# imperatormk/candle-birefnet

Measured on AMD Instinct MI355X. Metric: images/sec @1024x1024 Swin-L, higher is better.
Workload: dtype f32 storage+accumulate; GEMM operands as two fp16 planes of the power-of-two-scaled operand (22-bit mantissa), 3 fp16 MFMAs/product (fp32-equivalent inside the fp16 range: |GEMM input| < 8190); 1 GPU; BASELINE configs[1]: Swin-L 1024x1024 batch=1 fp32 on 1xMI355X (single-image latency); batch_per_gpu=1, global_batch=1, size=1024, deform_mode=reference_cpu, compute=f32_half2, streams_per_gpu=1, branch_streams_per_gpu=5, inputs=resident in HBM (torch cuda tensors), weights: synthetic seed 42

## Files before the change

candle_birefnet_amd/csrc/brn_graph_swin.cpp:

```cpp
#include "brn_graph.h"

namespace brn {

void swin_stage_dims(int H, int W, int patch, int hs[4], int ws[4]) {
    int h = (H + patch - 1) / patch, w = (W + patch - 1) / patch;
    for (int i = 0; i < 4; ++i) {
        hs[i] = h; ws[i] = w;
        h = (h + 1) / 2; w = (w + 1) / 2;
    }
}

static bool swin_attention_multi(Ctx& c, const SwinBlockW& blk, const float* xn, int B, int nin, const int* hs, const int* wsz, int C, int shift, float* y,
                                 const float* residual, int p2 = 0, int window = 12, const LNW* ln2 = nullptr, float* xn2 = nullptr, int ld_xn2 = 0) {
    const size_t mk = c.arena->mark();
    int M = 0;
    for (int k = 0; k < nin; ++k) M += B * hs[k] * wsz[k];
    float* qkv = c.act_alloc((size_t)M * 3 * C);
    const int ldp = p2 ? C * p2 / 2 : C;
    float* att = c.act_alloc((size_t)M * ldp);
    run_gemm(c, blk.qkv, GemmIO(xn, M, ldp).to(qkv, 3 * C).planes(p2, 0));
    if (!c.dry) {
        WindowAttnParams ps[2]{};
        size_t off = 0;
        double nwin = 0.0;
        for (int k = 0; k < nin; ++k) {
            WindowAttnParams& p = ps[k];
            p.qkv = c.at(qkv, off * 3 * C); p.qkv_bias = blk.qkv.bias; p.rel_table = blk.rel_table; p.out = c.at(att, off * ldp);
            p.io_bf16 = c.bf16;
            p.B = B; p.H = hs[k]; p.W = wsz[k]; p.C = C; p.heads = blk.heads;
            p.Hp = roundup(hs[k], window); p.Wp = roundup(wsz[k], window);
            p.ws = window;
            p.shift = shift; p.scale = 1.0f / sqrtf(32.0f);
            p.planes = (!c.bf16 && window == 12 && (blk.qkv.planes == 2 || blk.qkv.planes == 1)) ? blk.qkv.planes : 0;
            p.h2 = (p.planes == 2 && blk.qkv.half && switches().h2_att) ? 1 : 0;
            if (blk.qkv.half && !p.h2) p.planes = 0;
            p.out_planes = p2;
            p.out_h2 = (p2 == 2 && blk.qkv.half) ? c.h2_scale : 0.f;
            nwin += (double)B * (p.Hp / window) * (p.Wp / window) * blk.heads;
            off += (size_t)B * hs[k] * wsz[k];
        }
        const double ntok = (double)window * window;
        Bracket b(c, FAM_ATTENTION, nwin * 2.0 * 2.0 * ntok * ntok * 32, (double)c.esz() * ((double)M * 4 * C), M, C, shift);
        BRN_LAUNCH(launch_window_attention2(ps[0], nin > 1 ? &ps[1] : nullptr, c.stream));
    }
    bool ln_done = false;
    if (ln2 && xn2 && !p2 && y == residual) ln_done = linear_residual_ln(c, blk.proj, att, M, ldp, y, *ln2, xn2, ld_xn2);
    if (!ln_done) run_gemm(c, blk.proj, GemmIO(att, M, ldp).to(y, C).add(residual, C).planes(p2, 0).f32(c.bf16, c.bf16));
    c.arena->release(mk);
    return ln_done;
}

void swin_attention(Ctx& c, const SwinBlockW& blk, const float* xn, int B, int H, int W, int C, int shift, float* y, const float* residual, int window) {
    swin_attention_multi(c, blk, xn, B, 1, &H, &W, C, shift, y, residual, 0, window);
}

void swin_forward_multi(Ctx& c, const SwinW& w, const SwinIn* ins, int nin, int B, bool outs_f32) {
    if (nin < 1 || nin > 2) fail(BRN_ERR_INVALID_ARG, "swin_forward_multi: 1 or 2 inputs");
    int hs[2][4], wsz[2][4];
    for (int k = 0; k < nin; ++k) swin_stage_dims(ins[k].H, ins[k].W, w.patch, hs[k], wsz[k]);
    auto rows = [&](int k, int i) { return B * hs[k][i] * wsz[k][i]; };
    auto total = [&](int i) { int m = 0; for (int k = 0; k < nin; ++k) m += rows(k, i); return m; };
    const size_t mk0 = c.arena->mark();
    const int E = w.embed_dim;
    float* x = c.arena->alloc((size_t)total(0) * E);
    const int pe_env = switches().patch_ln;
    bool pe_fused = c.bf16 && pe_env != 0 && w.patch_proj.w && w.patch_proj.mode == GEMM_GATHER_NCHW && w.patch_proj.pad == 0 && w.patch_proj.dil == 1 &&
                    w.patch_proj.kh == w.patch_proj.kw && w.patch_norm.C == E && w.patch_norm.g && w.patch_norm.b;
    for (int k = 0; k < nin && pe_fused; ++k)
// ... 100 lines not shown
```

candle_birefnet_amd/csrc/brn_host.h:

```cpp
#pragma once
#include <hip/hip_runtime.h>
#include <stdint.h>
#include <stdarg.h>
#include <string>
#include <deque>
#include <vector>
#include <unordered_map>
#include <stdexcept>
#include <mutex>
#include <type_traits>
#include "../../include/birefnet_hip.h"
#include "brn_kernels.h"

namespace brn {

struct Error : std::runtime_error {
    int code;
    Error(int c, const std::string& m) : std::runtime_error(m), code(c) {}
};
[[noreturn]] void fail(int code, const char* fmt, ...);
void set_last_error(const std::string& s);
#define BRN_HIP(call)                                                                                   \
    do {                                                                                                \
        hipError_t e_ = (call);                                                                         \
// ... 34 lines not shown
    std::vector<hipEvent_t>* event_pool; size_t* event_next;
    int bf16 = 0;
    float h2_scale = 0.f;
    int region = REGION_NONE;
    BranchSet* br = nullptr;
    unsigned pending = 0;
    unsigned br_mask = ~0u;
    int esz() const { return bf16 ? 2 : 4; }
    float* act_alloc(size_t elems) { return arena->alloc_bytes(elems * (size_t)esz()); }
    template <class T> T* at(T* p, size_t elems) const { return reinterpret_cast<T*>(reinterpret_cast<char*>(const_cast<typename std::remove_const<T>::type*>(p)) + elems * (size_t)esz()); }
};

struct Map {
    float* p = nullptr;
    int B = 0, H = 0, W = 0, C = 0, ld = 0, coff = 0;
    Map() = default;
    Map(float* p_, int B_, int H_, int W_, int C_) : p(p_), B(B_), H(H_), W(W_), C(C_), ld(C_) {}
    size_t pixels() const { return (size_t)B * H * W; }
    Map window(int c0, int c) const { Map m = *this; m.coff = coff + c0; m.C = c; return m; }
};
Map new_map(Ctx& c, int B, int H, int W, int C);
static inline int roundup(int x, int m) { return (x + m - 1) / m * m; }

#define BRN_SWITCHES(X)                                                                                                                        \
    X(split_streams,    "BRN_SPLIT_STREAMS",     2,  "sub-batch streams of a device-resident batch (at least two images per part; 1 = one stream)") \
    X(branch_streams,   "BRN_BRANCH_STREAMS",    -1, "-1 = auxiliary branch streams when the batch is one part; 0 = none; else the mask forced (7 ASPP, 8 image-patch, 16 lateral)") \
    X(cu_partition,     "BRN_CU_PARTITION",      0,  "1 / 2 = two sub-batch streams confined to half the CUs of every XCD / to four XCDs each") \
    X(wstat,            "BRN_WSTAT",             3,  "mask of the K served by gemm_wstat_bf16_kernel (1 = 192, 2 = 384)")                     \
    X(wstat_ln,         "BRN_WSTAT_LN",          1,  "0 = stage-0 projection and norm2 as two launches instead of gemm_wstat_ln_bf16_kernel")   \
    X(rowln,            "BRN_ROWLN",             0,  "mask of the widths whose projection + LayerNorm run on gemm_rowln_bf16_kernel (1 = 768, 2 = 384)") \
    X(patch_ln,         "BRN_PATCH_LN",          1,  "0 = PatchEmbed as gather GEMM + LayerNorm in the 16-bit modes too; 2 = fused without the first block's norm1") \
    X(p1_f32,           "BRN_P1_F32",            1,  "0 = the decoder's last map p1 is a 16-bit map like every other in the 16-bit modes")     \
    X(h2_att,           "BRN_H2_ATT",            1,  "0 = mode f32_half2 runs the fp32-MFMA attention kernel instead of the fp16-pair one")     \
    X(h2_ascale,        "BRN_H2_ASCALE",         3,  "log2 of the scale of GEMM input activations before the fp16 split of mode f32_half2 (0 .. 8)") \
    X(deform_f32,       "BRN_DEFORM_F32_KERNEL", 0,  "1 = the 16-bit modes run deformable convolutions on the fp32-MFMA gather kernel")        \
    X(planes_kernel,    "BRN_PLANES_KERNEL",     0,  "1 = split modes with P-layout A on the LDS-DMA plane kernel (diag build only)")           \
    X(conv_chunk_major, "BRN_CONV_CHUNK_MAJOR",  1,  "0 = tap-major K order of the 16-bit implicit-GEMM conv weights (read when weights are packed)") \
    X(offmod_pad8,      "BRN_OFFMOD_PAD8",       1,  "0 = the offset / modulator conv's N padded to 4 instead of 8")
struct Switches {
#define BRN_X(field, name, dflt, doc) int field = dflt;
    BRN_SWITCHES(BRN_X)
#undef BRN_X
};
const Switches& switches();

constexpr int BUILD_BF16 = 16;
constexpr int BUILD_HALF2 = 18;
struct WeightBuild {
    int planes = 0;
    bool f16 = false;
};


struct GemmW {
    float* w = nullptr;
    void* wp = nullptr;
    int planes = 0, wp_rows = 0;
    int half = 0;
    float w_scale = 1.f;
    void* wb = nullptr;
    int wb_rows = 0, wb_ld = 0;
    int wb_chunk_major = 0;
    void* wf = nullptr;
    int N = 0, K = 0, Kreal = 0;
    int Cin = 0, Cinp = 0, kh = 1, kw = 1, stride = 1, pad = 0, dil = 1;
    int mode = GEMM_DENSE;
// ... 187 lines not shown
```

candle_birefnet_amd/csrc/brn_kernels.h:

```cpp
#pragma once
#include <hip/hip_runtime.h>
#include <stdint.h>

namespace brn {

enum GemmMode {
    GEMM_DENSE = 0,
    GEMM_CONV_NHWC = 1,
    GEMM_GATHER_NCHW = 2,
    GEMM_DEFORM_NHWC = 3
};
enum Act { ACT_NONE = 0, ACT_RELU = 1, ACT_GELU_ERF = 2 };

struct GemmParams {
    const float* A;
    const float* W;
    float* C;
    int M, N, K;
    int mode;
    int lda;
    int a_coff;
    int Hin, Win, Cin, kh, kw, stride, pad, dil, Hout, Wout;
    int Kreal;
    const float* om; int om_ld; int om_mask_off;
// ... 63 lines not shown
hipError_t launch_lds_mfma_probe(int blocks, int iters, int np, int variant, float* sink, hipStream_t s);
hipError_t launch_mfma_peak_bf16(int blocks, int iters, float* sink, unsigned long long* clk, int nacc, hipStream_t s);
hipError_t launch_mfma_peak(int blocks, int iters, float* sink, unsigned long long* clk, hipStream_t s);
#endif

struct LayerNormParams {
    const float* x; float* y;
    int rows, C;
    const float* gamma; const float* beta; float eps;
    int ldx;
    int ldy, y_coff;
    int mode; int H, W, Cin;
    int y_planes;
    float y_h2;
    int y_bf16;
};
hipError_t launch_layernorm(const LayerNormParams& p, hipStream_t s);

struct WindowAttnParams {
    const float* qkv;
    const float* qkv_bias;
    const float* rel_table;
    float* out;
    int B, H, W, C, heads;
    int Hp, Wp;
    int shift;
    float scale;
    int planes;
    int out_planes;
    int h2;
    float out_h2;
    int ws;
    int io_bf16;
};
hipError_t launch_window_attention(const WindowAttnParams& p, hipStream_t s);
hipError_t launch_window_attention2(const WindowAttnParams& p, const WindowAttnParams* p2, hipStream_t s);

hipError_t launch_resize_nhwc(const float* x, int B, int Hin, int Win, int C, int ldx, int x_coff,
                              float* y, int Hout, int Wout, int ldy, int y_coff, hipStream_t s, int bf16 = 0, int accumulate = 0);
hipError_t launch_resize_nchw(const float* x, int BC, int Hin, int Win, float* y, int Hout, int Wout, hipStream_t s);
hipError_t launch_nchw_to_nhwc(const float* x, int B, int C, int H, int W, float* y, int ldy, int y_coff, hipStream_t s, int bf16 = 0);
hipError_t launch_nhwc_to_nchw(const float* x, int B, int C, int H, int W, int ldx, int x_coff, float* y, hipStream_t s, int bf16 = 0);
hipError_t launch_image2patches(const float* x, int B, int Cimg, int H, int W, int th, int tw,
                                float* y, int ldy, int cpad, hipStream_t s, int bf16 = 0);
size_t gap_scratch_floats(int B, int HW, int C);
hipError_t launch_gap_nhwc(const float* x, int B, int HW, int C, int ldx, int x_coff, float* scratch, float* out, hipStream_t s, int bf16 = 0);
hipError_t launch_small_fc(const float* x, int B, int Cin, const float* w, int ldw, int w_off, int N,
                           const float* scale, const float* shift, int act, float* y, hipStream_t s);
hipError_t launch_gdt_gate(float* p, int npix, int C, int ldp, int p_coff, const float* g, int ldg,
                           const float* w, float bias, hipStream_t s, int bf16 = 0);
hipError_t launch_pixel_dot(const float* x, int npix, int C, int ldx, int x_coff, const float* w, float bias,
                            float* y, hipStream_t s, int bf16 = 0);
hipError_t launch_f32_to_bf16(const float* x, size_t n, float* y_bf16, hipStream_t s, int f16 = 0);
hipError_t launch_bf16_to_f32(const float* x_bf16, size_t n, float* y, hipStream_t s, int f16 = 0);
hipError_t launch_final_head(const float* q, int B, int h, int w, const float* t, float bias, int H, int W,
                             int apply_sigmoid, float* out, hipStream_t s);
hipError_t launch_head_stencil5x5(const float* img, int B, int H, int W, const float* k, const float* bias, float* y, hipStream_t s);
hipError_t launch_resample_v_u8(const unsigned char* in, int h, int w, int C, int nh, const int* left, const int* count,
                                const float* wts, int max_taps, float* out, hipStream_t s);
hipError_t launch_resample_h(const float* in, int nh, int w, int C, int nw, const int* left, const int* count, const float* wts,
                             int max_taps, unsigned char* out_u8, float* out_f32, const float* mean, const float* stdv, hipStream_t s);
hipError_t launch_mask_u8(const float* logits, long n, int apply_sigmoid, unsigned char* out, hipStream_t s);
hipError_t launch_sigmoid(const float* x, size_t n, float* y, hipStream_t s);
hipError_t launch_mod_sigmoid2(float* x, size_t rows, int ld, int c0, int c1, hipStream_t s);

}
// ... 1 lines not shown
```

candle_birefnet_amd/csrc/kernels/window_attention.hip:

```cpp
#include "../brn_kernels.h"
#include "split_planes.h"
#include <cstdlib>
#include <type_traits>

namespace brn {

typedef float f32x4 __attribute__((ext_vector_type(4)));

constexpr int WS = 12;
constexpr int NTOK = 144;
constexpr int HD = 32;
constexpr int KV_LD = 36;
constexpr int ATT_THREADS = 192;

template <int IOB>
__device__ __forceinline__ f32x4 att_load4(const float* base, long off) {
    if constexpr (IOB != 0) {
        using E = std::conditional_t<IOB == 2, _Float16, __bf16>;
        typedef E ex4_ld __attribute__((ext_vector_type(4)));
        const ex4_ld h = *reinterpret_cast<const ex4_ld*>(reinterpret_cast<const E*>(base) + off);
        return f32x4{(float)h[0], (float)h[1], (float)h[2], (float)h[3]};
    } else return *reinterpret_cast<const f32x4*>(base + off);
}
template <int IOB>
__device__ __forceinline__ f32x4 att_bias4(const float* bias) {
    f32x4 v = *reinterpret_cast<const f32x4*>(bias);
    if constexpr (IOB != 0) {
        using E = std::conditional_t<IOB == 2, _Float16, __bf16>;
#pragma unroll
        for (int e = 0; e < 4; ++e) v[e] = (float)(E)v[e];
    }
    return v;
}
template <int WSZ, int NWV = 3, int IOB = 0>
// ... 136 lines not shown
                o0 = __builtin_amdgcn_mfma_f32_16x16x4f32(vp[0], st[kt][r], o0, 0, 0, 0);
                o1 = __builtin_amdgcn_mfma_f32_16x16x4f32(vp[16], st[kt][r], o1, 0, 0, 0);
            }
            if (kt % 2 == 1) __builtin_amdgcn_sched_barrier(0);
        }
        if (qsrc >= 0 && qtok < NTOK) {
            const float inv = 1.0f / sum;
            if (p.out_planes == 3) {
                float* orow = p.out + (long)qsrc * (C + C / 2);
                store_planes<3>(orow, head * HD + g * 4, o0 * inv);
                store_planes<3>(orow, head * HD + 16 + g * 4, o1 * inv);
            } else if (p.out_planes == 2) {
                float* orow = p.out + (long)qsrc * C;
                store_planes_h(orow, head * HD + g * 4, o0 * inv, p.out_h2);
                store_planes_h(orow, head * HD + 16 + g * 4, o1 * inv, p.out_h2);
            } else if constexpr (IOB != 0) {
                using E = std::conditional_t<IOB == 2, _Float16, __bf16>;
                typedef E ex4_st __attribute__((ext_vector_type(4)));
                E* op = reinterpret_cast<E*>(p.out) + (long)qsrc * C + head * HD + g * 4;
                ex4_st h0, h1;
#pragma unroll
                for (int e = 0; e < 4; ++e) { h0[e] = (E)(o0[e] * inv); h1[e] = (E)(o1[e] * inv); }
                *reinterpret_cast<ex4_st*>(op) = h0;
                *reinterpret_cast<ex4_st*>(op + 16) = h1;
            } else {
                float* op = p.out + (long)qsrc * C + head * HD + g * 4;
                *reinterpret_cast<f32x4*>(op) = o0 * inv;
                *reinterpret_cast<f32x4*>(op + 16) = o1 * inv;
            }
        }
    }
}

typedef __bf16 bf16x8 __attribute__((ext_vector_type(8)));
typedef __bf16 bf16x4 __attribute__((ext_vector_type(4)));
typedef __bf16 bf16x2 __attribute__((ext_vector_type(2)));
constexpr int VT_LD = 148;

__device__ __forceinline__ int kswz(int key) { return (0x78 >> (2 * ((key >> 2) & 3))) & 3; }

constexpr float ATT_H_QKV = 8.0f, ATT_H_P = 2048.0f;
template <int NP, bool H = false>
__global__ void __launch_bounds__(ATT_THREADS) __attribute__((amdgpu_waves_per_eu(3, 3))) window_attention_split_kernel(const WindowAttnParams pa, const WindowAttnParams pb, const int nblk0) {
    static_assert(!H || NP == 2, "fp16 planes come in pairs");
    const bool second = (int)blockIdx.x >= nblk0;
    const WindowAttnParams& p = second ? pb : pa;
    __shared__ __attribute__((aligned(16))) __bf16 Kp[NP * NTOK * HD];
    __shared__ __attribute__((aligned(16))) __bf16 Vt[NP * HD * VT_LD];
    constexpr int TABN = (2 * WS - 1) * (2 * WS - 1);
    __shared__ float tab_s[TABN];
    __shared__ unsigned char rid_s[NTOK];
    __shared__ __attribute__((aligned(16))) float qb_s[HD];

    const int tid = threadIdx.x, lane = tid & 63, wave = tid >> 6;
    const int li = lane & 15, g = lane >> 4;
    const int head = blockIdx.y;
    const int nWw = p.Wp / WS, nW = (p.Hp / WS) * nWw;
    const int bw = second ? (int)blockIdx.x - nblk0 : (int)blockIdx.x;
    const int b = bw / nW, w = bw - b * nW;
    const int wr = w / nWw, wc = w - wr * nWw;
    const int C = p.C, C3 = 3 * C;
    const bool has_mask = p.shift > 0 && (wr == p.Hp / WS - 1 || wc == nWw - 1);

    auto tok_src = [&](int t) {
        const int ti = t / WS, tj = t - ti * WS;
        int sh = wr * WS + ti + p.shift, sw = wc * WS + tj + p.shift;
        if (sh >= p.Hp) sh -= p.Hp;
        if (sw >= p.Wp) sw -= p.Wp;
        return (sh < p.H && sw < p.W) ? (b * p.H + sh) * p.W + sw : -1;
    };
    static_assert((NTOK / 2) * 8 == 3 * ATT_THREADS && ATT_THREADS % 8 == 0 && 3 * ATT_THREADS >= TABN, "three staging items and three table words per thread");
    const int c4 = (tid & 7) * 4;
    const float* kbp = p.qkv_bias + C + head * HD + c4;
    const f32x4 kbias = *reinterpret_cast<const f32x4*>(kbp);
    const f32x4 vbias = *reinterpret_cast<const f32x4*>(kbp + C);
    f32x4 kvr[3][2], vvr[3][2];
    int ssrc[3][2];
#pragma unroll
    for (int it = 0; it < 3; ++it) {
#pragma unroll
        for (int u = 0; u < 2; ++u) {
            const int src = tok_src(((tid >> 3) + it * (ATT_THREADS / 8)) * 2 + u);
            ssrc[it][u] = src;
            const float* kp = p.qkv + (long)max(src, 0) * C3 + C + head * HD + c4;
            kvr[it][u] = *reinterpret_cast<const f32x4*>(kp);
            vvr[it][u] = *reinterpret_cast<const f32x4*>(kp + C);
        }
    }
    float tbw[3];
#pragma unroll
    for (int j = 0; j < 3; ++j) tbw[j] = p.rel_table[head * TABN + min(tid + j * ATT_THREADS, TABN - 1)];
    const float* qbp = p.qkv_bias + head * HD + g * 8;
    const f32x4 qbias0 = *reinterpret_cast<const f32x4*>(qbp);
    const f32x4 qbias1 = *reinterpret_cast<const f32x4*>(qbp + 4);
    int qsrc_n;
    f32x4 qn0, qn1;
    auto load_q = [&](int qtok) {
        qsrc_n = tok_src(qtok);
        const float* qp = p.qkv + (long)max(qsrc_n, 0) * C3 + head * HD + g * 8;
        qn0 = *reinterpret_cast<const f32x4*>(qp);
        qn1 = *reinterpret_cast<const f32x4*>(qp + 4);
    };
    load_q(wave * 16 + li);

    if (tid < NTOK) {
        const int ti = tid / WS, tj = tid - ti * WS;
        const int ph = wr * WS + ti, pw = wc * WS + tj;
        const int fh = ph < p.Hp - WS ? 0 : (ph < p.Hp - p.shift ? 1 : 2);
        const int fw = pw < p.Wp - WS ? 0 : (pw < p.Wp - p.shift ? 1 : 2);
        rid_s[tid] = (unsigned char)(fh * 3 + fw);
    }

#pragma unroll
    for (int it = 0; it < 3; ++it) {
        const int tp = (tid >> 3) + it * (ATT_THREADS / 8);
        f32x4 kv[2], vv[2];
#pragma unroll
        for (int u = 0; u < 2; ++u) {
            kv[u] = ssrc[it][u] < 0 ? kbias : kvr[it][u];
            vv[u] = ssrc[it][u] < 0 ? vbias : vvr[it][u];
        }
        if constexpr (H) {
#pragma unroll
            for (int u = 0; u < 2; ++u) {
                const int t = tp * 2 + u;
                bf16x4 sp[2];
                split4h<false>(kv[u], 0xffffffffu, ATT_H_QKV, sp);
#pragma unroll
                for (int pl = 0; pl < 2; ++pl)
                    *reinterpret_cast<bf16x4*>(Kp + (pl * NTOK + t) * HD + (((c4 >> 3) ^ kswz(t)) << 3) + (c4 & 4)) = sp[pl];
            }
// ... 13 lines not shown
            for (int pl = 0; pl < NP; ++pl) {
                bf16x4 h;
#pragma unroll
                for (int e = 0; e < 4; ++e) h[e] = (__bf16)r[e];
                *reinterpret_cast<bf16x4*>(Kp + (pl * NTOK + t) * HD + (((c4 >> 3) ^ kswz(t)) << 3) + (c4 & 4)) = h;
                if (pl + 1 < NP) {
#pragma unroll
                    for (int e = 0; e < 4; ++e) r[e] -= (float)h[e];
                }
            }
        }
        f32x4 r0 = vv[0], r1 = vv[1];
#pragma unroll
        for (int pl = 0; pl < NP; ++pl) {
#pragma unroll
            for (int e = 0; e < 4; ++e) {
                bf16x2 h;
                h[0] = (__bf16)r0[e]; h[1] = (__bf16)r1[e];
                *reinterpret_cast<bf16x2*>(Vt + (pl * HD + c4 + e) * VT_LD + tp * 2) = h;
                if (pl + 1 < NP) { r0[e] -= (float)h[0]; r1[e] -= (float)h[1]; }
            }
        }
        }
    }
#pragma unroll
    for (int j = 0; j < 3; ++j)
        if (tid + j * ATT_THREADS < TABN) tab_s[tid + j * ATT_THREADS] = tbw[j];
    if (tid < 64 && li == 0) {
        *reinterpret_cast<f32x4*>(qb_s + g * 8) = qbias0;
        *reinterpret_cast<f32x4*>(qb_s + g * 8 + 4) = qbias1;
    }
    __syncthreads();

    for (int qt = wave; qt < 9; qt += 3) {
        const int qtok = qt * 16 + li;
        const int qsrc = qsrc_n;
        const int qrid = rid_s[qtok];
        const int qbase = (qtok / WS + WS - 1) * (2 * WS - 1) + (qtok % WS) + WS - 1;
        bf16x8 qf[NP];
        {
            const f32x4 q0 = qsrc < 0 ? *reinterpret_cast<const f32x4*>(qb_s + g * 8) : qn0;
            const f32x4 q1 = qsrc < 0 ? *reinterpret_cast<const f32x4*>(qb_s + g * 8 + 4) : qn1;
            float r[8];
#pragma unroll
            for (int e = 0; e < 4; ++e) { r[e] = q0[e] * p.scale; r[4 + e] = q1[e] * p.scale; }
            if (qt + 3 < 9) load_q(qtok + 48);
            if constexpr (H) {
                typedef unsigned u32x4_q __attribute__((ext_vector_type(4)));
                u32x4_q hi, lo;
#pragma unroll
                for (int e = 0; e < 4; ++e) { unsigned a, b2; split_pair_h(r[2 * e], r[2 * e + 1], ATT_H_QKV, a, b2); hi[e] = a; lo[e] = b2; }
                qf[0] = __builtin_bit_cast(bf16x8, hi);
                qf[1] = __builtin_bit_cast(bf16x8, lo);
            } else {
#pragma unroll
            for (int pl = 0; pl < NP; ++pl) {
#pragma unroll
                for (int e = 0; e < 8; ++e) {
                    const __bf16 h = (__bf16)r[e];
                    qf[pl][e] = h;
                    r[e] -= (float)h;
                }
            }
            }
        }
        f32x4 st[9];
#pragma unroll
        for (int kt = 0; kt < 9; ++kt) {
            const int key = kt * 16 + li;
            bf16x8 kf[NP];
#pragma unroll
            for (int pl = 0; pl < NP; ++pl)
                kf[pl] = *reinterpret_cast<const bf16x8*>(Kp + (pl * NTOK + key) * HD + ((g ^ kswz(key)) << 3));
            f32x4 acc = {0.f, 0.f, 0.f, 0.f};
            if constexpr (H) {
                acc = __builtin_amdgcn_mfma_f32_16x16x32_f16(__builtin_bit_cast(f16x8, kf[1]), __builtin_bit_cast(f16x8, qf[0]), acc, 0, 0, 0);
                acc = __builtin_amdgcn_mfma_f32_16x16x32_f16(__builtin_bit_cast(f16x8, kf[0]), __builtin_bit_cast(f16x8, qf[1]), acc, 0, 0, 0);
                acc = __builtin_amdgcn_mfma_f32_16x16x32_f16(__builtin_bit_cast(f16x8, kf[0]), __builtin_bit_cast(f16x8, qf[0]), acc, 0, 0, 0);
            } else {
// ... 57 lines not shown
                        r[e] -= (float)h;
                    }
                }
                }
            }
#pragma unroll
            for (int dt = 0; dt < 2; ++dt) {
                bf16x8 vf[NP];
#pragma unroll
                for (int pl = 0; pl < NP; ++pl) {
                    const __bf16* vrow = Vt + (pl * HD + dt * 16 + li) * VT_LD + g * 4;
                    const bf16x4 lo = *reinterpret_cast<const bf16x4*>(vrow + (2 * t) * 16);
                    bf16x4 hi = {(__bf16)0.f, (__bf16)0.f, (__bf16)0.f, (__bf16)0.f};
                    if (2 * t + 1 < 9) hi = *reinterpret_cast<const bf16x4*>(vrow + (2 * t + 1) * 16);
#pragma unroll
                    for (int e = 0; e < 4; ++e) { vf[pl][e] = lo[e]; vf[pl][4 + e] = hi[e]; }
                }
                f32x4 o = dt == 0 ? o0 : o1;
                if constexpr (H) {
                    o = __builtin_amdgcn_mfma_f32_16x16x32_f16(__builtin_bit_cast(f16x8, vf[1]), __builtin_bit_cast(f16x8, pf[0]), o, 0, 0, 0);
                    o = __builtin_amdgcn_mfma_f32_16x16x32_f16(__builtin_bit_cast(f16x8, vf[0]), __builtin_bit_cast(f16x8, pf[1]), o, 0, 0, 0);
                    o = __builtin_amdgcn_mfma_f32_16x16x32_f16(__builtin_bit_cast(f16x8, vf[0]), __builtin_bit_cast(f16x8, pf[0]), o, 0, 0, 0);
                } else {
                if (NP == 2) {
                    o = __builtin_amdgcn_mfma_f32_16x16x32_bf16(vf[1], pf[0], o, 0, 0, 0);
                    o = __builtin_amdgcn_mfma_f32_16x16x32_bf16(vf[0], pf[1], o, 0, 0, 0);
                }
                o = __builtin_amdgcn_mfma_f32_16x16x32_bf16(vf[0], pf[0], o, 0, 0, 0);
                }
                if (dt == 0) o0 = o; else o1 = o;
            }
            __builtin_amdgcn_sched_barrier(0);
        }
        if (qsrc >= 0) {
            const float inv = (H ? 1.0f / (ATT_H_P * ATT_H_QKV) : 1.0f) / sum;
            if (H && p.out_planes == 2) {
                float* orow = p.out + (long)qsrc * C;
                store_planes_h(orow, head * HD + g * 4, o0 * inv, p.out_h2);
                store_planes_h(orow, head * HD + 16 + g * 4, o1 * inv, p.out_h2);
            } else if (p.out_planes == 2) {
                float* orow = p.out + (long)qsrc * C;
                store_planes<2>(orow, head * HD + g * 4, o0 * inv);
                store_planes<2>(orow, head * HD + 16 + g * 4, o1 * inv);
            } else {
                float* op = p.out + (long)qsrc * C + head * HD + g * 4;
                *reinterpret_cast<f32x4*>(op) = o0 * inv;
                *reinterpret_cast<f32x4*>(op + 16) = o1 * inv;
            }
        }
    }
}

__device__ __forceinline__ float max3f(float a, float b, float c) {
    float r;
    asm("v_max3_f32 %0, %1, %2, %3" : "=v"(r) : "v"(a), "v"(b), "v"(c));
    return r;
}
template <typename E>
__device__ __forceinline__ auto bias8_s16(const float* bp) {
    typedef E ex8_b __attribute__((ext_vector_type(8)));
    ex8_b r;
#pragma unroll
    for (int e = 0; e < 8; ++e) r[e] = (E)bp[e];
    return r;
}

template <int ATT_BF16_HPW, bool F16 = false>
__global__ void __launch_bounds__(ATT_BF16_HPW * ATT_THREADS) __attribute__((amdgpu_waves_per_eu(5, 8))) window_attention_bf16_kernel(const WindowAttnParams pa, const WindowAttnParams pb, const int nblk0) {
    using E = std::conditional_t<F16, _Float16, __bf16>;
    typedef E ex8 __attribute__((ext_vector_type(8)));
    typedef E ex4 __attribute__((ext_vector_type(4)));
    typedef E ex2 __attribute__((ext_vector_type(2)));
    auto mfma = [](const ex8 a, const ex8 b, const f32x4 c) -> f32x4 {
        if constexpr (F16) return __builtin_amdgcn_mfma_f32_16x16x32_f16(a, b, c, 0, 0, 0);
        else return __builtin_amdgcn_mfma_f32_16x16x32_bf16(a, b, c, 0, 0, 0);
    };
    const bool second = (int)blockIdx.x >= nblk0;
    const WindowAttnParams& p = second ? pb : pa;
    constexpr int TABN = (2 * WS - 1) * (2 * WS - 1);
    constexpr float LOG2E = 1.4426950408889634f;
    __shared__ __attribute__((aligned(16))) E Kp_[ATT_BF16_HPW][NTOK * HD];
    __shared__ __attribute__((aligned(16))) E Vt_[ATT_BF16_HPW][HD * VT_LD];
    __shared__ float rev_[ATT_BF16_HPW][TABN + 3];
    __shared__ __attribute__((aligned(4))) unsigned char rid_s[NTOK];

    const int tid = threadIdx.x, lane = tid & 63, wave = tid >> 6;
    const int hp = wave / 3, wv = wave - 3 * hp;
    const int head = blockIdx.y * ATT_BF16_HPW + hp;
    const int nWh = p.Hp / WS, nWw = p.Wp / WS, nW = nWh * nWw;
    const int bw = second ? (int)blockIdx.x - nblk0 : (int)blockIdx.x;
    const int b = bw / nW, w = bw - b * nW;
    const int wr = w / nWw, wc = w - wr * nWw;
    const int C = p.C, C3 = 3 * C;
    const E* qkv = reinterpret_cast<const E*>(p.qkv);
    const int li = lane & 15, g = lane >> 4;
    const bool has_mask = p.shift > 0 && (wr == nWh - 1 || wc == nWw - 1);
    E* Kp = Kp_[hp];
    E* Vt = Vt_[hp];
    const float* rev_s = rev_[hp];

    auto tok_src = [&](int t) {
        const int ti = t / WS, tj = t - ti * WS;
        int sh = wr * WS + ti + p.shift, sw = wc * WS + tj + p.shift;
        if (sh >= p.Hp) sh -= p.Hp;
        if (sw >= p.Wp) sw -= p.Wp;
        return (sh < p.H && sw < p.W) ? (b * p.H + sh) * p.W + sw : -1;
    };
    constexpr int NTHR = ATT_BF16_HPW * ATT_THREADS;
    constexpr int NITEM = (NTOK / 2) * 4 * ATT_BF16_HPW;
    constexpr int NTAB = ATT_BF16_HPW * TABN;
    static_assert(2 * NTHR >= NITEM && 3 * NTHR >= NTAB, "two staging items and three table words per thread cover a head group");
    ex8 qf[3];
    int qsrc_[3];
#pragma unroll
    for (int u = 0; u < 3; ++u) {
        const int qs = tok_src((wv + 3 * u) * 16 + li);
        qsrc_[u] = qs;
        qf[u] = *reinterpret_cast<const ex8*>(qkv + (long)max(qs, 0) * C3 + head * HD + g * 8);
    }
    float tbw[3];
#pragma unroll
    for (int j = 0; j < 3; ++j) {
        const int i = min(tid + j * NTHR, NTAB - 1), hh = i / TABN, jj = i - hh * TABN;
        tbw[j] = p.rel_table[(blockIdx.y * ATT_BF16_HPW + hh) * TABN + (TABN - 1 - jj)];
    }
    ex8 kv[2][2], vv[2][2];
    int ssrc[2][2];
#pragma unroll
    for (int it = 0; it < 2; ++it) {
        const int idx = min(tid + it * NTHR, NITEM - 1);
        const int c8 = (idx & 3) * 8, hh = (idx >> 2) & (ATT_BF16_HPW - 1), tp = idx / (4 * ATT_BF16_HPW);
        const int hd = (blockIdx.y * ATT_BF16_HPW + hh) * HD;
#pragma unroll
        for (int u = 0; u < 2; ++u) {
            const int src = tok_src(tp * 2 + u);
            ssrc[it][u] = src;
            const E* kp = qkv + (long)max(src, 0) * C3 + C + hd + c8;
            kv[it][u] = *reinterpret_cast<const ex8*>(kp);
            vv[it][u] = *reinterpret_cast<const ex8*>(kp + C);
        }
    }
    if (tid < NTOK) {
        const int ti = tid / WS, tj = tid - ti * WS;
        const int ph = wr * WS + ti, pw = wc * WS + tj;
        const int fh = ph < p.Hp - WS ? 0 : (ph < p.Hp - p.shift ? 1 : 2);
        const int fw = pw < p.Wp - WS ? 0 : (pw < p.Wp - p.shift ? 1 : 2);
        rid_s[tid] = (unsigned char)(fh * 3 + fw);
    }
#pragma unroll
    for (int j = 0; j < 3; ++j) {
        const int i = tid + j * NTHR;
        if (i < NTAB) { const int hh = i / TABN; rev_[hh][i - hh * TABN] = LOG2E * tbw[j]; }
    }
#pragma unroll
    for (int u = 0; u < 3; ++u)
        if (qsrc_[u] < 0) qf[u] = bias8_s16<E>(p.qkv_bias + head * HD + g * 8);
#pragma unroll
    for (int it = 0; it < 2; ++it) {
        const int idx = tid + it * NTHR;
        if (idx < NITEM) {
            const int c8 = (idx & 3) * 8, hh = (idx >> 2) & (ATT_BF16_HPW - 1), tp = idx / (4 * ATT_BF16_HPW);
            const int hd = (blockIdx.y * ATT_BF16_HPW + hh) * HD;
#pragma unroll
            for (int u = 0; u < 2; ++u) {
                if (ssrc[it][u] < 0) {
                    kv[it][u] = bias8_s16<E>(p.qkv_bias + C + hd + c8);
                    vv[it][u] = bias8_s16<E>(p.qkv_bias + 2 * C + hd + c8);
                }
            }
#pragma unroll
            for (int u = 0; u < 2; ++u) {
                const int t = tp * 2 + u;
                *reinterpret_cast<ex8*>(Kp_[hh] + t * HD + (((c8 >> 3) ^ kswz(t)) << 3)) = kv[it][u];
            }
#pragma unroll
            for (int e = 0; e < 8; ++e) {
                ex2 h;
                h[0] = vv[it][0][e]; h[1] = vv[it][1][e];
                *reinterpret_cast<ex2*>(Vt_[hh] + (c8 + e) * VT_LD + tp * 2) = h;
            }
        }
    }
    __syncthreads();

    const float scale2 = p.scale * LOG2E;
    ex8 ones8;
#pragma unroll
    for (int e = 0; e < 8; ++e) ones8[e] = (E)1.0f;
    typedef __attribute__((address_space(3))) const float lds_cfloat;
    unsigned koffb[9];
#pragma unroll
    for (int kt = 0; kt < 9; ++kt) { const int key0 = kt * 16 + g * 4; koffb[kt] = (unsigned)(key0 + 11 * (key0 / WS)) * 4u; }
#pragma unroll
    for (int u = 0; u < 3; ++u) {
        const int qt = wv + 3 * u;
        const int qtok = qt * 16 + li;
        const int qsrc = qsrc_[u];
        const unsigned qrid4 = 0x01010101u * (unsigned)rid_s[qtok];
        const int qrev = (TABN - 1) - ((qtok / WS + WS - 1) * (2 * WS - 1) + (qtok % WS) + WS - 1);
        f32x4 st[9];
#pragma unroll
        for (int kt = 0; kt < 9; ++kt) {
            const int key = kt * 16 + li;
            const ex8 kf = *reinterpret_cast<const ex8*>(Kp + key * HD + ((g ^ kswz(key)) << 3));
            f32x4 acc = {0.f, 0.f, 0.f, 0.f};
            st[kt] = mfma(kf, qf[u], acc);
            if (kt % 3 == 2) __builtin_amdgcn_sched_barrier(0);
        }
        float mx = -3.0e38f;
        unsigned tbq = (unsigned)(unsigned long)(lds_cfloat*)(rev_s + qrev);
        asm volatile("" : "+v"(tbq));
#pragma unroll
        for (int kt = 0; kt < 9; ++kt) {
            lds_cfloat* tb = (lds_cfloat*)(unsigned long)(tbq + koffb[kt]);
#pragma unroll
            for (int r = 0; r < 4; ++r) st[kt][r] = fmaf(st[kt][r], scale2, tb[r]);
        }
        if (has_mask) {
#pragma unroll
            for (int kt = 0; kt < 9; ++kt) {
                const unsigned xr = *reinterpret_cast<const unsigned*>(rid_s + kt * 16 + g * 4) ^ qrid4;
                const unsigned x = ((xr + 0x7f7f7f7fu) >> 7) & 0x01010101u;
#pragma unroll
                for (int r = 0; r < 4; ++r) st[kt][r] = fmaf((float)((x >> (8 * r)) & 0xffu), -100.0f * LOG2E, st[kt][r]);
            }
        }
#pragma unroll
        for (int kt = 0; kt < 9; ++kt) mx = max3f(max3f(mx, st[kt][0], st[kt][1]), st[kt][2], st[kt][3]);
        mx = fmaxf(mx, __shfl_xor(mx, 16));
        mx = fmaxf(mx, __shfl_xor(mx, 32));
#pragma unroll
        for (int kt = 0; kt < 9; ++kt) {
#pragma unroll
            for (int r = 0; r < 4; ++r) st[kt][r] = __builtin_amdgcn_exp2f(st[kt][r] - mx);
        }
        f32x4 o0 = {0.f, 0.f, 0.f, 0.f}, o1 = {0.f, 0.f, 0.f, 0.f}, osum = {0.f, 0.f, 0.f, 0.f};
#pragma unroll
        for (int t = 0; t < 5; ++t) {
            ex8 pf;
#pragma unroll
            for (int e = 0; e < 4; ++e) {
                pf[e] = (E)st[2 * t][e];
                pf[4 + e] = (2 * t + 1 < 9) ? (E)st[(2 * t + 1 < 9) ? 2 * t + 1 : 0][e] : (E)0.f;
            }
#pragma unroll
            for (int dt = 0; dt < 2; ++dt) {
                const E* vrow = Vt + (dt * 16 + li) * VT_LD + g * 4;
                const ex4 lo = *reinterpret_cast<const ex4*>(vrow + (2 * t) * 16);
                ex4 hi = {(E)0.f, (E)0.f, (E)0.f, (E)0.f};
                if (2 * t + 1 < 9) hi = *reinterpret_cast<const ex4*>(vrow + (2 * t + 1) * 16);
                ex8 vf;
#pragma unroll
                for (int e = 0; e < 4; ++e) { vf[e] = lo[e]; vf[4 + e] = hi[e]; }
                if (dt == 0) o0 = mfma(vf, pf, o0);
                else o1 = mfma(vf, pf, o1);
            }
            osum = mfma(ones8, pf, osum);
            __builtin_amdgcn_sched_barrier(0);
        }
        if (qsrc >= 0) {
            const float inv = __builtin_amdgcn_rcpf(osum[0]);
            E* op = reinterpret_cast<E*>(p.out) + (long)qsrc * C + head * HD + g * 4;
            ex4 h0, h1;
#pragma unroll
            for (int e = 0; e < 4; ++e) { h0[e] = (E)(o0[e] * inv); h1[e] = (E)(o1[e] * inv); }
            *reinterpret_cast<ex4*>(op) = h0;
            *reinterpret_cast<ex4*>(op + 16) = h1;
        }
    }
}

static hipError_t check_attention(const WindowAttnParams& p) {
    const int ws = p.ws ? p.ws : WS;
    if (!(ws == 12 || ws == 7)) return hipErrorInvalidValue;
    if (p.C != p.heads * HD || p.Hp % ws || p.Wp % ws || p.Hp < p.H || p.Wp < p.W) return hipErrorInvalidValue;
    if (!(p.shift == 0 || p.shift == ws / 2)) return hipErrorInvalidValue;
    if (ws != WS && (p.planes || p.out_planes)) return hipErrorInvalidValue;
    return hipSuccess;
}
hipError_t launch_window_attention2(const WindowAttnParams& p, const WindowAttnParams* p2, hipStream_t s) {
    if (check_attention(p) != hipSuccess) return hipErrorInvalidValue;
    const int ws = p.ws ? p.ws : WS;
    const int n0 = p.B * (p.Hp / ws) * (p.Wp / ws);
    int n1 = 0;
    if (p2) {
        if ((p2->ws ? p2->ws : WS) != ws) return hipErrorInvalidValue;
        if (check_attention(*p2) != hipSuccess || p2->C != p.C || p2->heads != p.heads || p2->planes != p.planes || p2->out_planes != p.out_planes || p2->io_bf16 != p.io_bf16) return hipErrorInvalidValue;
        n1 = p2->B * (p2->Hp / ws) * (p2->Wp / ws);
    }
    if (p.out_planes && !((p.out_planes == 2 && p.planes == 2 && (p.out_h2 > 0.f) == (p.h2 != 0)) || (p.out_planes == 3 && p.planes == 0) || (p.out_planes == 2 && p.planes == 0 && p.out_h2 > 0.f && !p.io_bf16)))
        return hipErrorInvalidValue;
    if (p.h2 && (p.planes != 2 || p.io_bf16)) return hipErrorInvalidValue;
    if (p2 && (p2->out_h2 != p.out_h2 || p2->h2 != p.h2)) return hipErrorInvalidValue;
    const WindowAttnParams& q = p2 ? *p2 : p;
    dim3 grid(n0 + n1, p.heads), block(ATT_THREADS);
    if (p.io_bf16 && ws == 7) {
        if (p.out_planes || (p.C & 3)) return hipErrorInvalidValue;
        if (p.io_bf16 == 2) hipLaunchKernelGGL((window_attention_f32_kernel<7, 3, 2>), grid, block, 0, s, p, q, n0);
        else hipLaunchKernelGGL((window_attention_f32_kernel<7, 3, 1>), grid, block, 0, s, p, q, n0);
    } else if (p.io_bf16) {
        if (p.out_planes || (p.C & 7)) return hipErrorInvalidValue;
        static const bool two_heads = !(getenv("BRN_ATT_HPW") && atoi(getenv("BRN_ATT_HPW")) == 1);
        if (p.io_bf16 == 2) {
            if (two_heads && !(p.heads & 1)) hipLaunchKernelGGL((window_attention_bf16_kernel<2, true>), dim3(n0 + n1, p.heads / 2), dim3(2 * ATT_THREADS), 0, s, p, q, n0);
            else hipLaunchKernelGGL((window_attention_bf16_kernel<1, true>), grid, block, 0, s, p, q, n0);
        } else if (two_heads && !(p.heads & 1)) hipLaunchKernelGGL(window_attention_bf16_kernel<2>, dim3(n0 + n1, p.heads / 2), dim3(2 * ATT_THREADS), 0, s, p, q, n0);
        else hipLaunchKernelGGL(window_attention_bf16_kernel<1>, grid, block, 0, s, p, q, n0);
    } else if (p.planes == 2 && p.h2) hipLaunchKernelGGL((window_attention_split_kernel<2, true>), grid, block, 0, s, p, q, n0);
    else if (p.planes == 2) hipLaunchKernelGGL(window_attention_split_kernel<2>, grid, block, 0, s, p, q, n0);
#ifdef BRN_DIAG_BUILD
    else if (p.planes == 1) hipLaunchKernelGGL(window_attention_split_kernel<1>, grid, block, 0, s, p, q, n0);
#else
    else if (p.planes == 1) return hipErrorInvalidValue;
#endif
    else if (ws == 7) hipLaunchKernelGGL(window_attention_f32_kernel<7>, grid, block, 0, s, p, q, n0);
    else {
        static const int f32_waves = getenv("BRN_ATT_F32_WAVES") ? atoi(getenv("BRN_ATT_F32_WAVES")) : 9;
        if (f32_waves == 9) hipLaunchKernelGGL((window_attention_f32_kernel<12, 9>), grid, dim3(9 * 64), 0, s, p, q, n0);
        else hipLaunchKernelGGL((window_attention_f32_kernel<12, 3>), grid, block, 0, s, p, q, n0);
    }
    return hipGetLastError();
}
hipError_t launch_window_attention(const WindowAttnParams& p, hipStream_t s) { return launch_window_attention2(p, nullptr, s); }

}
```

Before: 94.95 images/s.

## Skip padded query rows in window attention and order windows by work

Adds a window geometry helper that, for padded windows, maps query slots only onto real (non-padding) tokens. The split and bf16 attention kernels then run only as many 16-query tiles as there are real queries. The launcher also groups windows into classes by real-token count, sorts them heaviest first, and walks heads innermost, which should balance load across CUs. In exchange, every block pays extra index arithmetic (a class lookup and a division per slot token) and the kernels carry more code.

```diff
diff --git a/candle_birefnet_amd/csrc/brn_graph_swin.cpp b/candle_birefnet_amd/csrc/brn_graph_swin.cpp
--- a/candle_birefnet_amd/csrc/brn_graph_swin.cpp
+++ b/candle_birefnet_amd/csrc/brn_graph_swin.cpp
@@ -34,6 +34,7 @@
             p.planes = (!c.bf16 && window == 12 && (blk.qkv.planes == 2 || blk.qkv.planes == 1)) ? blk.qkv.planes : 0;
             p.h2 = (p.planes == 2 && blk.qkv.half && switches().h2_att) ? 1 : 0;
             if (blk.qkv.half && !p.h2) p.planes = 0;
+            p.pack_q = switches().att_pack_q;
             p.out_planes = p2;
             p.out_h2 = (p2 == 2 && blk.qkv.half) ? c.h2_scale : 0.f;
             nwin += (double)B * (p.Hp / window) * (p.Wp / window) * blk.heads;
diff --git a/candle_birefnet_amd/csrc/brn_host.h b/candle_birefnet_amd/csrc/brn_host.h
--- a/candle_birefnet_amd/csrc/brn_host.h
+++ b/candle_birefnet_amd/csrc/brn_host.h
@@ -90,6 +90,7 @@
     X(patch_ln,         "BRN_PATCH_LN",          1,  "0 = PatchEmbed as gather GEMM + LayerNorm in the 16-bit modes too; 2 = fused without the first block's norm1") \
     X(p1_f32,           "BRN_P1_F32",            1,  "0 = the decoder's last map p1 is a 16-bit map like every other in the 16-bit modes")     \
     X(h2_att,           "BRN_H2_ATT",            1,  "0 = mode f32_half2 runs the fp32-MFMA attention kernel instead of the fp16-pair one")     \
+    X(att_pack_q,       "BRN_ATT_PACK_Q",        1,  "0 = the split / bf16 attention kernels compute the pad queries too, windows in grid order; 2 = real queries only, grid order") \
     X(h2_ascale,        "BRN_H2_ASCALE",         3,  "log2 of the scale of GEMM input activations before the fp16 split of mode f32_half2 (0 .. 8)") \
     X(deform_f32,       "BRN_DEFORM_F32_KERNEL", 0,  "1 = the 16-bit modes run deformable convolutions on the fp32-MFMA gather kernel")        \
     X(planes_kernel,    "BRN_PLANES_KERNEL",     0,  "1 = split modes with P-layout A on the LDS-DMA plane kernel (diag build only)")           \
diff --git a/candle_birefnet_amd/csrc/brn_kernels.h b/candle_birefnet_amd/csrc/brn_kernels.h
--- a/candle_birefnet_amd/csrc/brn_kernels.h
+++ b/candle_birefnet_amd/csrc/brn_kernels.h
@@ -119,6 +119,7 @@
     float out_h2;
     int ws;
     int io_bf16;
+    int pack_q;
 };
 hipError_t launch_window_attention(const WindowAttnParams& p, hipStream_t s);
 hipError_t launch_window_attention2(const WindowAttnParams& p, const WindowAttnParams* p2, hipStream_t s);
diff --git a/candle_birefnet_amd/csrc/kernels/window_attention.hip b/candle_birefnet_amd/csrc/kernels/window_attention.hip
--- a/candle_birefnet_amd/csrc/kernels/window_attention.hip
+++ b/candle_birefnet_amd/csrc/kernels/window_attention.hip
@@ -1,5 +1,6 @@
 #include "../brn_kernels.h"
 #include "split_planes.h"
+#include "window_geometry.h"
 #include <cstdlib>
 #include <type_traits>
 
@@ -202,6 +203,19 @@
     }
 }
 
+struct AttBlock { WindowId win; int head; };
+__device__ __forceinline__ AttBlock att_block(const WindowOrder& ord) {
+    int flat = blockIdx.x, head = blockIdx.y;
+    if (ord.heads_inner) {
+        const int f = blockIdx.y * gridDim.x + blockIdx.x;
+        flat = f / (int)gridDim.y;
+        head = f - flat * (int)gridDim.y;
+    }
+    AttBlock r;
+    r.win = order_window(ord, flat);
+    r.head = head;
+    return r;
+}
 typedef __bf16 bf16x8 __attribute__((ext_vector_type(8)));
 typedef __bf16 bf16x4 __attribute__((ext_vector_type(4)));
 typedef __bf16 bf16x2 __attribute__((ext_vector_type(2)));
@@ -211,9 +225,10 @@
 
 constexpr float ATT_H_QKV = 8.0f, ATT_H_P = 2048.0f;
 template <int NP, bool H = false>
-__global__ void __launch_bounds__(ATT_THREADS) __attribute__((amdgpu_waves_per_eu(3, 3))) window_attention_split_kernel(const WindowAttnParams pa, const WindowAttnParams pb, const int nblk0) {
+__global__ void __launch_bounds__(ATT_THREADS) __attribute__((amdgpu_waves_per_eu(3, 3))) window_attention_split_kernel(const WindowAttnParams pa, const WindowAttnParams pb, const WindowOrder ord) {
     static_assert(!H || NP == 2, "fp16 planes come in pairs");
-    const bool second = (int)blockIdx.x >= nblk0;
+    const AttBlock blk = att_block(ord);
+    const bool second = blk.win.geom != 0;
     const WindowAttnParams& p = second ? pb : pa;
     __shared__ __attribute__((aligned(16))) __bf16 Kp[NP * NTOK * HD];
     __shared__ __attribute__((aligned(16))) __bf16 Vt[NP * HD * VT_LD];
@@ -224,12 +239,12 @@
 
     const int tid = threadIdx.x, lane = tid & 63, wave = tid >> 6;
     const int li = lane & 15, g = lane >> 4;
-    const int head = blockIdx.y;
-    const int nWw = p.Wp / WS, nW = (p.Hp / WS) * nWw;
-    const int bw = second ? (int)blockIdx.x - nblk0 : (int)blockIdx.x;
-    const int b = bw / nW, w = bw - b * nW;
-    const int wr = w / nWw, wc = w - wr * nWw;
+    const int head = blk.head;
+    const int nWw = p.Wp / WS;
+    const int b = blk.win.b, wr = blk.win.wr, wc = blk.win.wc;
     const int C = p.C, C3 = 3 * C;
+    const WindowReal wg = window_real(wr, wc, p.shift, p.H, p.W, p.Hp, p.Wp, ord.pack != 0);
+    const int nq = wg.nq, ntile = window_tiles(wg);
     const bool has_mask = p.shift > 0 && (wr == p.Hp / WS - 1 || wc == nWw - 1);
 
     auto tok_src = [&](int t) {
@@ -263,10 +278,11 @@
     const float* qbp = p.qkv_bias + head * HD + g * 8;
     const f32x4 qbias0 = *reinterpret_cast<const f32x4*>(qbp);
     const f32x4 qbias1 = *reinterpret_cast<const f32x4*>(qbp + 4);
-    int qsrc_n;
+    int qsrc_n, qtok_n;
     f32x4 qn0, qn1;
-    auto load_q = [&](int qtok) {
-        qsrc_n = tok_src(qtok);
+    auto load_q = [&](int slot) {
+        qtok_n = slot_token(wg, min(slot, nq - 1));
+        qsrc_n = tok_src(qtok_n);
         const float* qp = p.qkv + (long)max(qsrc_n, 0) * C3 + head * HD + g * 8;
         qn0 = *reinterpret_cast<const f32x4*>(qp);
         qn1 = *reinterpret_cast<const f32x4*>(qp + 4);
@@ -346,8 +362,9 @@
     }
     __syncthreads();
 
-    for (int qt = wave; qt < 9; qt += 3) {
-        const int qtok = qt * 16 + li;
+    for (int qt = wave; qt < ntile; qt += 3) {
+        const int slot = qt * 16 + li;
+        const int qtok = qtok_n;
         const int qsrc = qsrc_n;
         const int qrid = rid_s[qtok];
         const int qbase = (qtok / WS + WS - 1) * (2 * WS - 1) + (qtok % WS) + WS - 1;
@@ -358,7 +375,7 @@
             float r[8];
 #pragma unroll
             for (int e = 0; e < 4; ++e) { r[e] = q0[e] * p.scale; r[4 + e] = q1[e] * p.scale; }
-            if (qt + 3 < 9) load_q(qtok + 48);
+            if (qt + 3 < ntile) load_q(slot + 48);
             if constexpr (H) {
                 typedef unsigned u32x4_q __attribute__((ext_vector_type(4)));
                 u32x4_q hi, lo;
@@ -482,7 +499,7 @@
             }
             __builtin_amdgcn_sched_barrier(0);
         }
-        if (qsrc >= 0) {
+        if (qsrc >= 0 && slot < nq) {
             const float inv = (H ? 1.0f / (ATT_H_P * ATT_H_QKV) : 1.0f) / sum;
             if (H && p.out_planes == 2) {
                 float* orow = p.out + (long)qsrc * C;
@@ -516,7 +533,7 @@
 }
 
 template <int ATT_BF16_HPW, bool F16 = false>
-__global__ void __launch_bounds__(ATT_BF16_HPW * ATT_THREADS) __attribute__((amdgpu_waves_per_eu(5, 8))) window_attention_bf16_kernel(const WindowAttnParams pa, const WindowAttnParams pb, const int nblk0) {
+__global__ void __launch_bounds__(ATT_BF16_HPW * ATT_THREADS) __attribute__((amdgpu_waves_per_eu(5, 8))) window_attention_bf16_kernel(const WindowAttnParams pa, const WindowAttnParams pb, const WindowOrder ord) {
     using E = std::conditional_t<F16, _Float16, __bf16>;
     typedef E ex8 __attribute__((ext_vector_type(8)));
     typedef E ex4 __attribute__((ext_vector_type(4)));
@@ -525,7 +542,8 @@
         if constexpr (F16) return __builtin_amdgcn_mfma_f32_16x16x32_f16(a, b, c, 0, 0, 0);
         else return __builtin_amdgcn_mfma_f32_16x16x32_bf16(a, b, c, 0, 0, 0);
     };
-    const bool second = (int)blockIdx.x >= nblk0;
+    const AttBlock blk = att_block(ord);
+    const bool second = blk.win.geom != 0;
     const WindowAttnParams& p = second ? pb : pa;
     constexpr int TABN = (2 * WS - 1) * (2 * WS - 1);
     constexpr float LOG2E = 1.4426950408889634f;
@@ -536,12 +554,12 @@
 
     const int tid = threadIdx.x, lane = tid & 63, wave = tid >> 6;
     const int hp = wave / 3, wv = wave - 3 * hp;
-    const int head = blockIdx.y * ATT_BF16_HPW + hp;
-    const int nWh = p.Hp / WS, nWw = p.Wp / WS, nW = nWh * nWw;
-    const int bw = second ? (int)blockIdx.x - nblk0 : (int)blockIdx.x;
-    const int b = bw / nW, w = bw - b * nW;
-    const int wr = w / nWw, wc = w - wr * nWw;
+    const int head0 = blk.head * ATT_BF16_HPW, head = head0 + hp;
+    const int nWh = p.Hp / WS, nWw = p.Wp / WS;
+    const int b = blk.win.b, wr = blk.win.wr, wc = blk.win.wc;
     const int C = p.C, C3 = 3 * C;
+    const WindowReal wg = window_real(wr, wc, p.shift, p.H, p.W, p.Hp, p.Wp, ord.pack != 0);
+    const int nq = wg.nq, ntile = window_tiles(wg);
     const E* qkv = reinterpret_cast<const E*>(p.qkv);
     const int li = lane & 15, g = lane >> 4;
     const bool has_mask = p.shift > 0 && (wr == nWh - 1 || wc == nWw - 1);
@@ -564,7 +582,7 @@
     int qsrc_[3];
 #pragma unroll
     for (int u = 0; u < 3; ++u) {
-        const int qs = tok_src((wv + 3 * u) * 16 + li);
+        const int qs = tok_src(slot_token(wg, min((wv + 3 * u) * 16 + li, nq - 1)));
         qsrc_[u] = qs;
         qf[u] = *reinterpret_cast<const ex8*>(qkv + (long)max(qs, 0) * C3 + head * HD + g * 8);
     }
@@ -572,7 +590,7 @@
 #pragma unroll
     for (int j = 0; j < 3; ++j) {
         const int i = min(tid + j * NTHR, NTAB - 1), hh = i / TABN, jj = i - hh * TABN;
-        tbw[j] = p.rel_table[(blockIdx.y * ATT_BF16_HPW + hh) * TABN + (TABN - 1 - jj)];
+        tbw[j] = p.rel_table[(head0 + hh) * TABN + (TABN - 1 - jj)];
     }
     ex8 kv[2][2], vv[2][2];
     int ssrc[2][2];
@@ -580,7 +598,7 @@
     for (int it = 0; it < 2; ++it) {
         const int idx = min(tid + it * NTHR, NITEM - 1);
         const int c8 = (idx & 3) * 8, hh = (idx >> 2) & (ATT_BF16_HPW - 1), tp = idx / (4 * ATT_BF16_HPW);
-        const int hd = (blockIdx.y * ATT_BF16_HPW + hh) * HD;
+        const int hd = (head0 + hh) * HD;
 #pragma unroll
         for (int u = 0; u < 2; ++u) {
             const int src = tok_src(tp * 2 + u);
@@ -610,7 +628,7 @@
         const int idx = tid + it * NTHR;
         if (idx < NITEM) {
             const int c8 = (idx & 3) * 8, hh = (idx >> 2) & (ATT_BF16_HPW - 1), tp = idx / (4 * ATT_BF16_HPW);
-            const int hd = (blockIdx.y * ATT_BF16_HPW + hh) * HD;
+            const int hd = (head0 + hh) * HD;
 #pragma unroll
             for (int u = 0; u < 2; ++u) {
                 if (ssrc[it][u] < 0) {
@@ -644,7 +662,9 @@
 #pragma unroll
     for (int u = 0; u < 3; ++u) {
         const int qt = wv + 3 * u;
-        const int qtok = qt * 16 + li;
+        if (qt >= ntile) break;
+        const int slot = qt * 16 + li;
+        const int qtok = slot_token(wg, min(slot, nq - 1));
         const int qsrc = qsrc_[u];
         const unsigned qrid4 = 0x01010101u * (unsigned)rid_s[qtok];
         const int qrev = (TABN - 1) - ((qtok / WS + WS - 1) * (2 * WS - 1) + (qtok % WS) + WS - 1);
@@ -708,7 +728,7 @@
             osum = mfma(ones8, pf, osum);
             __builtin_amdgcn_sched_barrier(0);
         }
-        if (qsrc >= 0) {
+        if (qsrc >= 0 && slot < nq) {
             const float inv = __builtin_amdgcn_rcpf(osum[0]);
             E* op = reinterpret_cast<E*>(p.out) + (long)qsrc * C + head * HD + g * 4;
             ex4 h0, h1;
@@ -744,6 +764,11 @@
     if (p2 && (p2->out_h2 != p.out_h2 || p2->h2 != p.h2)) return hipErrorInvalidValue;
     const WindowAttnParams& q = p2 ? *p2 : p;
     dim3 grid(n0 + n1, p.heads), block(ATT_THREADS);
+    WindowOrder ord;
+    {
+        const WindowGeom g[2] = {{p.B, p.H, p.W, p.Hp, p.Wp, p.shift}, {q.B, q.H, q.W, q.Hp, q.Wp, q.shift}};
+        build_window_order(g, p2 ? 2 : 1, ws == WS && p.pack_q != 0, p.pack_q != 2, ord);
+    }
     if (p.io_bf16 && ws == 7) {
         if (p.out_planes || (p.C & 3)) return hipErrorInvalidValue;
         if (p.io_bf16 == 2) hipLaunchKernelGGL((window_attention_f32_kernel<7, 3, 2>), grid, block, 0, s, p, q, n0);
@@ -752,14 +777,14 @@
         if (p.out_planes || (p.C & 7)) return hipErrorInvalidValue;
         static const bool two_heads = !(getenv("BRN_ATT_HPW") && atoi(getenv("BRN_ATT_HPW")) == 1);
         if (p.io_bf16 == 2) {
-            if (two_heads && !(p.heads & 1)) hipLaunchKernelGGL((window_attention_bf16_kernel<2, true>), dim3(n0 + n1, p.heads / 2), dim3(2 * ATT_THREADS), 0, s, p, q, n0);
-            else hipLaunchKernelGGL((window_attention_bf16_kernel<1, true>), grid, block, 0, s, p, q, n0);
-        } else if (two_heads && !(p.heads & 1)) hipLaunchKernelGGL(window_attention_bf16_kernel<2>, dim3(n0 + n1, p.heads / 2), dim3(2 * ATT_THREADS), 0, s, p, q, n0);
-        else hipLaunchKernelGGL(window_attention_bf16_kernel<1>, grid, block, 0, s, p, q, n0);
-    } else if (p.planes == 2 && p.h2) hipLaunchKernelGGL((window_attention_split_kernel<2, true>), grid, block, 0, s, p, q, n0);
-    else if (p.planes == 2) hipLaunchKernelGGL(window_attention_split_kernel<2>, grid, block, 0, s, p, q, n0);
+            if (two_heads && !(p.heads & 1)) hipLaunchKernelGGL((window_attention_bf16_kernel<2, true>), dim3(n0 + n1, p.heads / 2), dim3(2 * ATT_THREADS), 0, s, p, q, ord);
+            else hipLaunchKernelGGL((window_attention_bf16_kernel<1, true>), grid, block, 0, s, p, q, ord);
+        } else if (two_heads && !(p.heads & 1)) hipLaunchKernelGGL(window_attention_bf16_kernel<2>, dim3(n0 + n1, p.heads / 2), dim3(2 * ATT_THREADS), 0, s, p, q, ord);
+        else hipLaunchKernelGGL(window_attention_bf16_kernel<1>, grid, block, 0, s, p, q, ord);
+    } else if (p.planes == 2 && p.h2) hipLaunchKernelGGL((window_attention_split_kernel<2, true>), grid, block, 0, s, p, q, ord);
+    else if (p.planes == 2) hipLaunchKernelGGL(window_attention_split_kernel<2>, grid, block, 0, s, p, q, ord);
 #ifdef BRN_DIAG_BUILD
-    else if (p.planes == 1) hipLaunchKernelGGL(window_attention_split_kernel<1>, grid, block, 0, s, p, q, n0);
+    else if (p.planes == 1) hipLaunchKernelGGL(window_attention_split_kernel<1>, grid, block, 0, s, p, q, ord);
 #else
     else if (p.planes == 1) return hipErrorInvalidValue;
 #endif
diff --git a/candle_birefnet_amd/csrc/kernels/window_geometry.h b/candle_birefnet_amd/csrc/kernels/window_geometry.h
--- /dev/null
+++ b/candle_birefnet_amd/csrc/kernels/window_geometry.h
@@ -0,0 +1,129 @@
+#pragma once
+#include <climits>
+
+#if defined(__HIPCC__)
+#define BRN_WG_HD __host__ __device__ __forceinline__
+#else
+#define BRN_WG_HD inline
+#endif
+
+namespace brn {
+
+constexpr int WG_WS = 12;
+constexpr int WG_NTOK = WG_WS * WG_WS;
+
+BRN_WG_HD int wg_min(int a, int b) { return a < b ? a : b; }
+BRN_WG_HD int wg_max(int a, int b) { return a > b ? a : b; }
+
+struct AxisReal { int n, split, gap; };
+
+BRN_WG_HD AxisReal axis_real(int w, int shift, int L, int Lp) {
+    const int s = w * WG_WS + shift;
+    const int n1 = wg_max(0, wg_min(s + WG_WS, L) - s);
+    const int lo2 = wg_max(s, Lp);
+    const int n2 = wg_max(0, wg_min(s + WG_WS, Lp + L) - lo2);
+    AxisReal a;
+    a.n = n1 + n2; a.split = n1; a.gap = n2 > 0 ? lo2 - s - n1 : 0;
+    return a;
+}
+BRN_WG_HD int axis_coord(const AxisReal& a, int k) { return k + (k >= a.split ? a.gap : 0); }
+
+struct WindowReal {
+    AxisReal r, c;
+    int nq;
+    int cdiv;
+};
+BRN_WG_HD WindowReal window_real(int wr, int wc, int shift, int H, int W, int Hp, int Wp, bool pack) {
+    WindowReal g;
+    if (pack) { g.r = axis_real(wr, shift, H, Hp); g.c = axis_real(wc, shift, W, Wp); }
+    else { g.r.n = WG_WS; g.r.split = WG_WS; g.r.gap = 0; g.c = g.r; }
+    g.nq = g.r.n * g.c.n;
+    g.cdiv = (65536 + g.c.n - 1) / g.c.n;
+    return g;
+}
+BRN_WG_HD int window_tiles(const WindowReal& g) { return (g.nq + 15) >> 4; }
+BRN_WG_HD int slot_token(const WindowReal& g, int slot) {
+    const int q = (slot * g.cdiv) >> 16, r = slot - q * g.c.n;
+    return axis_coord(g.r, q) * WG_WS + axis_coord(g.c, r);
+}
+
+constexpr int WG_MAX_CLS = 18;
+struct WindowClass { int geom, wr0, nwr, wc0, nwc, tiles; };
+struct WindowOrder {
+    int pack;
+    int heads_inner;
+    int ncls;
+    int start[WG_MAX_CLS];
+    WindowClass cls[WG_MAX_CLS];
+};
+struct WindowId { int geom, b, wr, wc; };
+BRN_WG_HD WindowId order_window(const WindowOrder& o, int flat) {
+    int ci = 0;
+    for (int i = 1; i < WG_MAX_CLS; ++i) ci += (int)((unsigned)(o.start[i] - flat - 1) >> 31);
+    const WindowClass& k = o.cls[ci];
+    const int l = flat - o.start[ci], per = k.nwr * k.nwc;
+    WindowId id;
+    id.geom = k.geom;
+    id.b = l / per;
+    const int r = l - id.b * per, rr = r / k.nwc;
+    id.wr = k.wr0 + rr;
+    id.wc = k.wc0 + (r - rr * k.nwc);
+    return id;
+}
+
+struct WindowGeom { int B, H, W, Hp, Wp, shift; };
+inline void identity_window_order(const WindowGeom* g, int ngeom, WindowOrder& o) {
+    o.pack = 0; o.heads_inner = 0; o.ncls = ngeom;
+    int at = 0;
+    for (int i = 0; i < WG_MAX_CLS; ++i) {
+        o.start[i] = INT_MAX;
+        o.cls[i] = WindowClass{0, 0, 1, 0, 1, 0};
+        if (i < ngeom) {
+            o.start[i] = at;
+            o.cls[i] = WindowClass{i, 0, g[i].Hp / WG_WS, 0, g[i].Wp / WG_WS, WG_NTOK / 16};
+            at += g[i].B * (g[i].Hp / WG_WS) * (g[i].Wp / WG_WS);
+        }
+    }
+}
+inline void build_window_order(const WindowGeom* g, int ngeom, bool pack, bool reorder, WindowOrder& o) {
+    identity_window_order(g, ngeom, o);
+    bool padded = false;
+    for (int k = 0; k < ngeom; ++k) padded = padded || g[k].Hp != g[k].H || g[k].Wp != g[k].W;
+    if (!pack || !padded) return;
+    o.pack = 1;
+    if (!reorder) return;
+    WindowClass cls[WG_MAX_CLS];
+    int ncls = 0;
+    for (int k = 0; k < ngeom; ++k) {
+        const int nWh = g[k].Hp / WG_WS, nWw = g[k].Wp / WG_WS, shift = g[k].shift;
+        for (int r0 = 0; r0 < nWh;) {
+            const int nr = axis_real(r0, shift, g[k].H, g[k].Hp).n;
+            int r1 = r0 + 1;
+            while (r1 < nWh && axis_real(r1, shift, g[k].H, g[k].Hp).n == nr) ++r1;
+            for (int c0 = 0; c0 < nWw;) {
+                const int nc = axis_real(c0, shift, g[k].W, g[k].Wp).n;
+                int c1 = c0 + 1;
+                while (c1 < nWw && axis_real(c1, shift, g[k].W, g[k].Wp).n == nc) ++c1;
+                if (ncls == WG_MAX_CLS) return;
+                cls[ncls++] = WindowClass{k, r0, r1 - r0, c0, c1 - c0, (nr * nc + 15) >> 4};
+                c0 = c1;
+            }
+            r0 = r1;
+        }
+    }
+    for (int i = 1; i < ncls; ++i) {
+        const WindowClass c = cls[i];
+        int j = i;
+        for (; j > 0 && cls[j - 1].tiles < c.tiles; --j) cls[j] = cls[j - 1];
+        cls[j] = c;
+    }
+    o.heads_inner = 1; o.ncls = ncls;
+    int at = 0;
+    for (int i = 0; i < ncls; ++i) {
+        o.start[i] = at;
+        o.cls[i] = cls[i];
+        at += g[cls[i].geom].B * cls[i].nwr * cls[i].nwc;
+    }
+}
+
+}
```

After: 96.18 images/s (median of 6 runs). +1.3%, better.
